# pansanity666/TransHuman

Measured on AMD Instinct MI355X. Metric: rays/sec (512x512, 64 samples/ray), higher is better.
Workload: dtype f32 (fp16 hi/lo x3 MFMA emulation)

## Files before the change

transhuman_amd/csrc/k_mlp_fused8_kernel.h:

```cpp
#pragma once
#include "k_mlp_fused_kernel.h"

typedef float f8_f4 __attribute__((ext_vector_type(4)));
typedef short f8_s4 __attribute__((ext_vector_type(4)));
typedef short f8_s8 __attribute__((ext_vector_type(8)));

#define F8_THREADS 512
#define F8_PART_FLOATS (3 * 8 * 32)
#define F8_PSTR 12
#define F8_MISC_FLOATS (F8_PSTR * 32 + F8_PART_FLOATS + 32 + 8)
#define F8_LDS_BYTES (ABUF_BYTES + MBUF_BYTES + F8_MISC_FLOATS * 4)
static_assert(F8_LDS_BYTES <= 163840, "the 8-wave tile must fit the CU's LDS");

#define F8_MFMA(A, B, C) __builtin_amdgcn_mfma_f32_16x16x32_f16((A), (B), (C), 0, 0, 0)

template <int CT>
__device__ __forceinline__ void f8_load_w(const uint4* __restrict__ wl, int t, uint4 (&w)[CT][2]) {
    const uint4* p = wl + (long long)t * (CT * 2 * 64);
#pragma unroll
    for (int c = 0; c < CT; ++c) {
        w[c][0] = p[(c * 2 + 0) * 64];
        w[c][1] = p[(c * 2 + 1) * 64];
    }
}
#define F8_WSLICE(L, wave, ct) ((L).w + (long long)(wave) * (L).KB * ((ct) * 2 * 64))

template <int NR, int ROWSTEP, bool PERM>
__device__ __forceinline__ void f8_load_x(const char* __restrict__ ahi, const char* __restrict__ alo, int aoff, int t,
                                          h8 (&xh)[NR], h8 (&xl)[NR]) {
    const int ko = (PERM ? 32 : 64) * t;
#pragma unroll
    for (int r = 0; r < NR; ++r) {
        xh[r] = *reinterpret_cast<const h8*>(ahi + r * ROWSTEP + aoff + ko);
        xl[r] = *reinterpret_cast<const h8*>(alo + r * ROWSTEP + aoff + ko);
    }
}
template <bool PERM>
__device__ __forceinline__ int f8_aoff(int lane, int str) {
    const int l = lane & 15, g = lane >> 4;
    return PERM ? l * str + 16 * (g >> 1) + 256 * (g & 1) : l * str + 16 * g;
}

template <int CT, int RT, int NR, int R0, bool FIRST>
__device__ __forceinline__ void f8_mfma_half(const uint4 (&w)[CT][2], const h8 (&xh)[NR], const h8 (&xl)[NR], f8_f4 (&acc)[CT][RT]) {
    const f8_f4 zero = {0.f, 0.f, 0.f, 0.f};
#pragma unroll
    for (int c = 0; c < CT; ++c)
#pragma unroll
        for (int r = 0; r < NR; ++r)
            acc[c][R0 + r] = F8_MFMA(*reinterpret_cast<const h8*>(&w[c][1]), xh[r], FIRST ? zero : acc[c][R0 + r]);
#pragma unroll
    for (int c = 0; c < CT; ++c)
#pragma unroll
        for (int r = 0; r < NR; ++r) acc[c][R0 + r] = F8_MFMA(*reinterpret_cast<const h8*>(&w[c][0]), xl[r], acc[c][R0 + r]);
#pragma unroll
    for (int c = 0; c < CT; ++c)
#pragma unroll
        for (int r = 0; r < NR; ++r) acc[c][R0 + r] = F8_MFMA(*reinterpret_cast<const h8*>(&w[c][0]), xh[r], acc[c][R0 + r]);
}

template <int NMEM, int NMF>
__device__ __forceinline__ void f8_interleave() {
    constexpr int NP = NMEM < NMF ? NMEM : NMF;
#pragma unroll
    for (int q = 0; q < NP; ++q) {
        __builtin_amdgcn_sched_group_barrier(0x008, 1, 0);
        __builtin_amdgcn_sched_group_barrier(0x120, 1, 0);
    }
    if constexpr (NMF > NP) __builtin_amdgcn_sched_group_barrier(0x008, NMF - NP, 0);
    if constexpr (NMEM > NP) __builtin_amdgcn_sched_group_barrier(0x120, NMEM - NP, 0);
    FM_SB();
}

template <int RT, int CT, int ROWSTEP, bool PERM, bool PRE = false>
__device__ __forceinline__ void f8_gemm(const char* __restrict__ ahi, const char* __restrict__ alo, int str,
                                        const uint4* __restrict__ wp, int T, int lane, f8_f4 (&acc)[CT][RT], uint4 (&w)[2][CT][2]) {
    static_assert(RT % 2 == 0, "row tiles come in halves");
    constexpr int NR = RT / 2;
    const uint4* wl = wp + lane;
    const int aoff = f8_aoff<PERM>(lane, str);
    h8 xah[NR], xal[NR], xbh[NR], xbl[NR];
    if (!PRE) f8_load_w<CT>(wl, 0, w[0]);
    f8_load_x<NR, ROWSTEP, PERM>(ahi, alo, aoff, 0, xah, xal);
    FM_SB();
    auto step = [&](auto first, auto par, int t) __attribute__((always_inline)) {
        constexpr bool F = decltype(first)::value;
        constexpr int PB = decltype(par)::value;
        const int tn = t + 1 < T ? t + 1 : T - 1;
        f8_load_x<NR, ROWSTEP, PERM>(ahi + NR * ROWSTEP, alo + NR * ROWSTEP, aoff, t, xbh, xbl);
        f8_load_w<CT>(wl, tn, w[PB ^ 1]);
        f8_mfma_half<CT, RT, NR, 0, F>(w[PB], xah, xal, acc);
        f8_interleave<2 * NR + 2 * CT, 3 * CT * NR>();
        f8_load_x<NR, ROWSTEP, PERM>(ahi, alo, aoff, tn, xah, xal);
        f8_mfma_half<CT, RT, NR, NR, F>(w[PB], xbh, xbl, acc);
        f8_interleave<2 * NR, 3 * CT * NR>();
    };
    step(std::true_type{}, std::integral_constant<int, 0>{}, 0);
    if (T > 1) {
        step(std::false_type{}, std::integral_constant<int, 1>{}, 1);
#pragma unroll 1
        for (int t = 2; t < T; t += 2) {
            step(std::false_type{}, std::integral_constant<int, 0>{}, t);
            step(std::false_type{}, std::integral_constant<int, 1>{}, t + 1);
        }
    }
}

template <int RT, int CT, int ROWSTEP, bool PERM, bool PRE = false>
__device__ __forceinline__ void f8_gemm3(const char* __restrict__ ahi, const char* __restrict__ alo, int str,
                                         const uint4* __restrict__ wp, int T, int lane, f8_f4 (&acc)[CT][RT], uint4 (&w)[2][CT][2]) {
    static_assert(RT % 3 == 0, "row tiles come in thirds");
    constexpr int NR = RT / 3;
    const uint4* wl = wp + lane;
    const int aoff = f8_aoff<PERM>(lane, str);
    h8 xh[2][NR], xl[2][NR];
    if (!PRE) f8_load_w<CT>(wl, 0, w[0]);
    f8_load_x<NR, ROWSTEP, PERM>(ahi, alo, aoff, 0, xh[0], xl[0]);
    FM_SB();
    auto sub = [&](auto first, auto sidx, int t) __attribute__((always_inline)) {
        constexpr int S = decltype(sidx)::value, G = S % 3, PB = S / 3, CUR = S & 1;
        constexpr bool F = decltype(first)::value && S < 3;
        constexpr int GN = (G + 1) % 3;
        const int tt = t + PB;
        const int tx = G == 2 ? (tt + 1 < T ? tt + 1 : T - 1) : tt;
        f8_load_x<NR, ROWSTEP, PERM>(ahi + GN * NR * ROWSTEP, alo + GN * NR * ROWSTEP, aoff, tx, xh[CUR ^ 1], xl[CUR ^ 1]);
        if constexpr (G == 0) f8_load_w<CT>(wl, tt + 1 < T ? tt + 1 : T - 1, w[PB ^ 1]);
        f8_mfma_half<CT, RT, NR, G * NR, F>(w[PB], xh[CUR], xl[CUR], acc);
        f8_interleave<2 * NR + (G == 0 ? 2 * CT : 0), 3 * CT * NR>();
    };
    auto pair = [&](auto first, int t) __attribute__((always_inline)) {
        sub(first, std::integral_constant<int, 0>{}, t); sub(first, std::integral_constant<int, 1>{}, t);
        sub(first, std::integral_constant<int, 2>{}, t); sub(first, std::integral_constant<int, 3>{}, t);
        sub(first, std::integral_constant<int, 4>{}, t); sub(first, std::integral_constant<int, 5>{}, t);
    };
    pair(std::true_type{}, 0);
#pragma unroll 1
    for (int t = 2; t < T; t += 2) pair(std::false_type{}, t);
}
template <int RT, int CT, int ROWSTEP, bool PERM, bool PRE = false>
__device__ __forceinline__ void f8_gemm_rt(const char* __restrict__ ahi, const char* __restrict__ alo, int str,
                                           const uint4* __restrict__ wp, int T, int lane, f8_f4 (&acc)[CT][RT], uint4 (&w)[2][CT][2]) {
    if constexpr (RT % 3 == 0) f8_gemm3<RT, CT, ROWSTEP, PERM, PRE>(ahi, alo, str, wp, T, lane, acc, w);
    else f8_gemm<RT, CT, ROWSTEP, PERM, PRE>(ahi, alo, str, wp, T, lane, acc, w);
}

template <int STR, bool NONNEG = true>
__device__ __forceinline__ void f8_store_h(const f8_f4& t, int row, int col0, char* __restrict__ hi, char* __restrict__ lo, int lane,
                                           unsigned& rm) {
    const int c = col0 + 4 * (lane >> 4);
    uint2 a, b;
    split_pair(t[0], t[1], a.x, b.x);
    split_pair(t[2], t[3], a.y, b.y);
    range_acc<NONNEG>(rm, a.x);
    range_acc<NONNEG>(rm, a.y);
    *reinterpret_cast<uint2*>(hi + row * STR + 2 * c) = a;
    *reinterpret_cast<uint2*>(lo + row * STR + 2 * c) = b;
}
__device__ __forceinline__ f8_f4 f8_finish(const f8_f4& a, const float4& b, float inv_scale, bool relu) {
    const f32x2 sc = {inv_scale, inv_scale};
    f32x2 y01 = __builtin_elementwise_fma((f32x2){a[0], a[1]}, sc, (f32x2){b.x, b.y});
    f32x2 y23 = __builtin_elementwise_fma((f32x2){a[2], a[3]}, sc, (f32x2){b.z, b.w});
    if (relu) {
        y01 = __builtin_elementwise_max(y01, (f32x2){0.f, 0.f});
        y23 = __builtin_elementwise_max(y23, (f32x2){0.f, 0.f});
    }
    return (f8_f4){y01[0], y01[1], y23[0], y23[1]};
}
__device__ __forceinline__ float f8_xor(float v, int lane, int mask) {
    return __builtin_bit_cast(float, __builtin_amdgcn_ds_bpermute((lane ^ mask) << 2, __builtin_bit_cast(int, v)));
}
__device__ __forceinline__ float4 f8_bias(const float* __restrict__ bias, int col0, int lane) {
    return *reinterpret_cast<const float4*>(bias + col0 + 4 * (lane >> 4));
}

template <int RT, int NV, int H, int R0, bool FIRST>
__device__ __forceinline__ void f8_mfma_dual(const uint4 (&r3)[2][2], const uint4 (&ra)[1][2], const h8 (&mh)[1], const h8 (&ml)[1],
                                             const h8 (&xh)[NV], const h8 (&xl)[NV], f8_f4 (&a3)[2][2], f8_f4 (&va)[1][RT]) {
    const f8_f4 zero = {0.f, 0.f, 0.f, 0.f};
#pragma unroll
    for (int t = 0; t < 3; ++t) {
        const int wp = t == 0 ? 1 : 0;
        const bool lo = t == 1;
        const bool first = FIRST && t == 0;
        a3[0][H] = F8_MFMA(*reinterpret_cast<const h8*>(&r3[0][wp]), lo ? ml[0] : mh[0], first ? zero : a3[0][H]);
#pragma unroll
        for (int r = 0; r < NV; ++r) {
            va[0][R0 + r] = F8_MFMA(*reinterpret_cast<const h8*>(&ra[0][wp]), lo ? xl[r] : xh[r], first ? zero : va[0][R0 + r]);
            if (r == 0) a3[1][H] = F8_MFMA(*reinterpret_cast<const h8*>(&r3[1][wp]), lo ? ml[0] : mh[0], first ? zero : a3[1][H]);
        }
    }
}

template <int V>
__global__ __launch_bounds__(F8_THREADS, 2) void mlp_fused8_kernel(FusedParams P_arg) {
#define PK P_arg
    struct F8Dbg { long long* dbg; };
    const F8Dbg P{PK.dbg};
    extern __shared__ __attribute__((aligned(16))) char lds[];
    char* abuf = lds;
    char* mbuf = lds + ABUF_BYTES;
    float* misc = reinterpret_cast<float*>(lds + ABUF_BYTES + MBUF_BYTES);
    float* probs = misc;
    float* part = misc + F8_PSTR * 32;
    float* sig = part + F8_PART_FLOATS;
    int* flag = reinterpret_cast<int*>(sig + 32);

    const int tid = threadIdx.x, lane = tid & 63, wave = tid >> 6;
    const int l15 = lane & 15, g4 = lane >> 4;
    const int tile = (int)((blockIdx.x & 7) * (gridDim.x >> 3) + (blockIdx.x >> 3));
    const int pbase = tile * FM_PTS;
    if (pbase >= PK.P) return;
    const int npts = min(FM_PTS, PK.P - pbase);
    const int fm_dbg_tile = tile;
    const int zoff = 0;
    constexpr int ROWS = 32 * V, RT = 2 * V;
    constexpr int RS256 = 16 * STR256;
    int dbg_i = 1;
    long long dbg_t = 0;
    long long* dbg_keep = reinterpret_cast<long long*>(flag + 2);
    constexpr float inv_v = 1.0f / (float)V;
    unsigned rmax = 0u;
    unsigned seen_s = 0u, seen_p = 0u, seen_n = 0u, seen_i = 0u, seen_4 = 0u;
    char* a256_lo = abuf + ROWS * STR256;

    struct TexPre { unsigned h0, h1; fm_u4 rq; };
    auto tex_fetch = [&]() __attribute__((always_inline)) {
        int tl = tile;
        asm volatile("" : "+s"(tl));
        TexPre t;
        const unsigned* hb = PK.tex_hdr + (long long)tl * 512;
        t.h0 = hb[lane];
        t.h1 = hb[64 + lane];
        t.rq = (fm_u4){0u, 0u, 0u, 0u};
        if (tid < 64 * V) t.rq = *reinterpret_cast<const fm_u4*>(PK.tex_rec + (long long)tl * V * 32 * 8 + tid * 4);
        return t;
    };
    auto fill_tex = [&](const TexPre& pre, auto rgb, auto&& under) __attribute__((always_inline)) {
        constexpr bool RGB = decltype(rgb)::value;
        constexpr int TSTR = 1040, TMAX = 103, NK = (TMAX + 7) / 8, NR = 4 * V;
        static_assert(TMAX * TSTR <= ABUF_BYTES, "a pass of texel rows must fit the operand buffer");
        int wv = __builtin_amdgcn_readfirstlane(wave), tl = tile;
        asm volatile("" : "+s"(wv), "+s"(tl));
        const unsigned* hb = PK.tex_hdr + (long long)tl * 512;
        unsigned h0 = pre.h0, h1 = pre.h1;
        const int npass = __builtin_amdgcn_readfirstlane((int)(h0 >> 16));
        char* recl = reinterpret_cast<char*>(misc);
        static_assert(32 * V * 32 <= (F8_PSTR * 32 + F8_PART_FLOATS) * 4, "row records must fit probs + part");
        unsigned fv[NR][4] = {};
        f32x2 bias_lo = {0.f, 0.f}, bias_hi = {0.f, 0.f};
        if constexpr (!RGB) {
            const float4 b4 = *reinterpret_cast<const float4*>(PK.ar0.bias + 4 * lane);
            bias_lo = (f32x2){b4.x, b4.y};
            bias_hi = (f32x2){b4.z, b4.w};
        }
        for (int p = 0; p < npass; ++p) {
            if (p > 0) {
                FM_SYNCL();
                h0 = hb[p * 128 + lane];
                h1 = hb[p * 128 + 64 + lane];
            }
            const int U = __builtin_amdgcn_readfirstlane((int)(h0 & 0xffffu));
            {
                constexpr int NA = 7, NB = 10;
                const char* mbase = reinterpret_cast<const char*>(RGB ? PK.tex_map2 : PK.tex_map);
                const unsigned loff = (unsigned)lane * 16u;
                const int last = U - 1;
                fm_u4 ta[NA], tb[NB - NA], tc[NK - NB];
#pragma unroll
                for (int k = 0; k < NA; ++k) {
                    const int i = min(wv + 8 * k, last);
                    const unsigned id = (unsigned)__builtin_amdgcn_readlane((int)h0, 8 + i);
                    ta[k] = *reinterpret_cast<const fm_u4*>(mbase + TX_ADDR(id));
                }
                const bool more = U > 8 * NA, most = U > 8 * NB;
                if (more) {
#pragma unroll
                    for (int k = NA; k < NB; ++k) {
                        const int i = min(wv + 8 * k, last);
                        const unsigned id = (unsigned)__builtin_amdgcn_readlane((int)h1, i - 56);
                        tb[k - NA] = *reinterpret_cast<const fm_u4*>(mbase + TX_ADDR(id));
                    }
                }
                if (most) {
#pragma unroll
                    for (int k = NB; k < NK; ++k) {
                        const int i = min(wv + 8 * k, last);
                        const unsigned id = (unsigned)__builtin_amdgcn_readlane((int)h1, i - 56);
                        tc[k - NB] = *reinterpret_cast<const fm_u4*>(mbase + TX_ADDR(id));
                    }
                }
                if (p == 0) {
                    under();
                    if (tid < 64 * V) *reinterpret_cast<fm_u4*>(recl + tid * 16) = pre.rq;
                }
                int wv2 = wv;
                asm volatile("" : "+s"(wv2));
#pragma unroll
                for (int k = 0; k < NA; ++k) *reinterpret_cast<fm_u4*>(abuf + min(wv2 + 8 * k, last) * TSTR + lane * 16) = ta[k];
                if (more) {
#pragma unroll
                    for (int k = NA; k < NB; ++k) *reinterpret_cast<fm_u4*>(abuf + min(wv2 + 8 * k, last) * TSTR + lane * 16) = tb[k - NA];
                }
                if (most) {
#pragma unroll
                    for (int k = NB; k < NK; ++k) *reinterpret_cast<fm_u4*>(abuf + min(wv2 + 8 * k, last) * TSTR + lane * 16) = tc[k - NB];
                }
            }
            FM_SYNCL();
            const int sh2 = npass == 1 ? 2 : npass == 2 ? 1 : 0;
            const int cofs = lane * 16;
            struct RowIn { float4 a, b, c, d; fm_u4 q0; };
            auto issue = [&](int k, const fm_u4& o, RowIn& r) __attribute__((always_inline)) {
                r.q0 = *reinterpret_cast<const fm_u4*>(recl + (wv + 8 * k) * 32);
                r.a = *reinterpret_cast<const float4*>(abuf + (o[0] + cofs));
                r.b = *reinterpret_cast<const float4*>(abuf + (o[1] + cofs));
                r.c = *reinterpret_cast<const float4*>(abuf + (o[2] + cofs));
                r.d = *reinterpret_cast<const float4*>(abuf + (o[3] + cofs));
            };
            auto offs = [&](int k) __attribute__((always_inline)) {
                return *reinterpret_cast<const fm_u4*>(recl + (wv + 8 * k) * 32 + 16);
            };
            auto blend = [&](int k, const RowIn& r, auto sel) __attribute__((always_inline)) {
                const unsigned u0 = r.q0[0], u1 = r.q0[1], u2 = r.q0[2], u3 = r.q0[3];
                const float w00 = __builtin_bit_cast(float, u0), w01 = __builtin_bit_cast(float, u1),
                            w10 = __builtin_bit_cast(float, u2), w11 = __builtin_bit_cast(float, u3);
                const f32x2 W00 = {w00, w00}, W01 = {w01, w01}, W10 = {w10, w10}, W11 = {w11, w11};
                f32x2 lo = (f32x2){r.a.x, r.a.y} * W00, hi = (f32x2){r.a.z, r.a.w} * W00;
                lo = __builtin_elementwise_fma((f32x2){r.b.x, r.b.y}, W01, lo);
                hi = __builtin_elementwise_fma((f32x2){r.b.z, r.b.w}, W01, hi);
                lo = __builtin_elementwise_fma((f32x2){r.c.x, r.c.y}, W10, lo);
                hi = __builtin_elementwise_fma((f32x2){r.c.z, r.c.w}, W10, hi);
                lo = __builtin_elementwise_fma((f32x2){r.d.x, r.d.y}, W11, lo);
                hi = __builtin_elementwise_fma((f32x2){r.d.z, r.d.w}, W11, hi);
                unsigned n0, n1, n2, n3;
                if constexpr (RGB) {
                    const float l0 = lo[0], l1 = lo[1], h0f = hi[0], h1f = hi[1];
                    n0 = __builtin_bit_cast(unsigned, l0); n1 = __builtin_bit_cast(unsigned, l1);
                    n2 = __builtin_bit_cast(unsigned, h0f); n3 = __builtin_bit_cast(unsigned, h1f);
                } else {
                    lo = __builtin_elementwise_max(lo + bias_lo, (f32x2){0.f, 0.f});
                    hi = __builtin_elementwise_max(hi + bias_hi, (f32x2){0.f, 0.f});
                    split_pair(lo[0], lo[1], n0, n2);
                    split_pair(hi[0], hi[1], n1, n3);
                }
                if constexpr (decltype(sel)::value) {
                    const bool mine = ((k & 3) >> sh2) == p;
                    fv[k][0] = mine ? n0 : fv[k][0]; fv[k][1] = mine ? n1 : fv[k][1];
                    fv[k][2] = mine ? n2 : fv[k][2]; fv[k][3] = mine ? n3 : fv[k][3];
                } else {
                    fv[k][0] = n0; fv[k][1] = n1; fv[k][2] = n2; fv[k][3] = n3;
                }
            };
            auto rows_loop = [&](auto sel) __attribute__((always_inline)) {
                RowIn in[2];
                fm_u4 of[2];
                of[0] = offs(0);
                of[1] = offs(1);
                issue(0, of[0], in[0]);
#pragma unroll
                for (int k = 0; k < NR; ++k) {
                    if (k + 1 < NR) issue(k + 1, of[(k + 1) & 1], in[(k + 1) & 1]);
                    if (k + 2 < NR) of[k & 1] = offs(k + 2);
                    FM_SB();
                    blend(k, in[k & 1], sel);
                    FM_SB();
                }
            };
            if (npass == 1) rows_loop(std::false_type{});
            else rows_loop(std::true_type{});
        }
        FM_SYNCL();
        if constexpr (RGB) {
#pragma unroll
            for (int k = 0; k < NR; ++k)
                *reinterpret_cast<fm_u4*>(abuf + (wv + 8 * k) * TSTR + lane * 16) = (fm_u4){fv[k][0], fv[k][1], fv[k][2], fv[k][3]};
        } else {
#pragma unroll
            for (int k = 0; k < NR; ++k) {
                range_acc<true>(rmax, fv[k][0]);
                range_acc<true>(rmax, fv[k][1]);
                *reinterpret_cast<uint2*>(abuf + (wv + 8 * k) * STR256 + lane * 8) = make_uint2(fv[k][0], fv[k][1]);
                *reinterpret_cast<uint2*>(a256_lo + (wv + 8 * k) * STR256 + lane * 8) = make_uint2(fv[k][2], fv[k][3]);
            }
            range_commit(PK.range, TH_RANGE_P, seen_p, rmax);
        }
    };

    if (PK.dbg != nullptr && tid == 0 && (tile & 15) == 0) {
        atomicAdd(reinterpret_cast<unsigned long long*>(PK.dbg), 1ull);
        dbg_t = clock64();
        dbg_keep[0] = dbg_t;
        dbg_keep[1] = wall_clock64();
    }
    fm_u4 rv4 = {0u, 0u, 0u, 0u};
    unsigned rv1 = 0u;
    static_assert(TH_RANGE_S == 1 && TH_RANGE_P == 2 && TH_RANGE_N == 3 && TH_RANGE_INTER == 4 && TH_RANGE_F4 == 5, "range slots 1..5");
    if (PK.range != nullptr) {
        const unsigned* rtab = PK.range + zoff;
        rv4 = (fm_u4){rtab[1], rtab[2], rtab[3], rtab[4]};
        rv1 = rtab[5];
    }
    TexPre tex_pre = tex_fetch(), tex_pre2;

    int vsel[2] = {0, 0};
    float vdv[2] = {0.f, 0.f};
    f8_f4 acc2[2][RT];
    {
        constexpr int STOK_STR = 1040;
        static_assert(32 * V * STOK_STR <= ABUF_BYTES, "T' rows must fit the operand buffer");
        char* pe_hi = mbuf;
        char* pe_lo = mbuf + 32 * STR64;
        const int pt = tid & 255, prow = pt >> 3, pc = pt & 7, ppl = tid >> 8;
        const int psrc = min(prow, npts - 1);
        const uint4 pe_v = *reinterpret_cast<const uint4*>(PK.pe + (long long)(pbase + psrc) * 128 + 64 * ppl + 8 * pc);
        char* wsp_hi = mbuf + 16384;
        char* wsp_lo = wsp_hi + 32 * STRVD;
        const unsigned* hdr = reinterpret_cast<const unsigned*>(PK.stok) + (long long)((PK.P + 31) / 32 * 32) * 16 + (long long)tile * 128;
        const unsigned h0 = hdr[lane], h1 = hdr[64 + lane];
        const int ns = tid / 7, nk = tid - 7 * ns;
        int slot = -1;
        float nw = 0.f;
        if (tid < 224) {
            const unsigned* rec = reinterpret_cast<const unsigned*>(PK.stok) + (long long)(pbase + min(ns, npts - 1)) * 16;
            slot = (int)rec[nk];
            nw = __builtin_bit_cast(float, rec[8 + nk]);
        }
        const unsigned zq = 0u;
        const float inv_t = PK.t_inv[zoff];
        uint4 wq[2][2][2];
        const uint4* wl = F8_WSLICE(PK.w16.fc_0pe, wave, 2) + lane;
        f8_load_w<2>(wl, 0, wq[0]);
        f8_load_w<2>(wl, 1, wq[1]);
        const float4 b0[2] = {f8_bias(PK.fc_0pe.bias, wave * 32, lane), f8_bias(PK.fc_0pe.bias, wave * 32 + 16, lane)};
        if (tid < 2 * 32 * STRVD / 16) reinterpret_cast<uint4*>(wsp_hi)[tid] = make_uint4(zq, zq, zq, zq);
        *reinterpret_cast<uint4*>((ppl ? pe_lo : pe_hi) + prow * STR64 + 16 * pc) = pe_v;
        const int U = __builtin_amdgcn_readfirstlane((int)h0);
        FM_SB();
        auto slot_centre = [&](int u) {
            const int d = (2 + u) >> 1;
            const unsigned src = d < 64 ? (unsigned)__builtin_amdgcn_readlane((int)h0, d) : (unsigned)__builtin_amdgcn_readlane((int)h1, d - 64);
            return (int)((src >> (16 * ((2 + u) & 1))) & 0xffffu);
        };
#pragma unroll
        for (int c = 0; c < 2; ++c)
#pragma unroll
            for (int r = 0; r < RT; ++r) acc2[c][r] = (f8_f4){0.f, 0.f, 0.f, 0.f};
        f8_f4 a1[2][2] = {{{0.f, 0.f, 0.f, 0.f}, {0.f, 0.f, 0.f, 0.f}}, {{0.f, 0.f, 0.f, 0.f}, {0.f, 0.f, 0.f, 0.f}}};
        const int wv = __builtin_amdgcn_readfirstlane(wave);
        const int aoffw = f8_aoff<false>(lane, STRVD), aoffp = f8_aoff<false>(lane, STR64);
        for (int u0 = 0; u0 < U; u0 += 32) {
            const int nU = min(32, U - u0);
            if (u0 > 0) {
                FM_SYNCL();
                if (tid < 2 * 32 * STRVD / 16) reinterpret_cast<uint4*>(wsp_hi)[tid] = make_uint4(zq, zq, zq, zq);
            }
            for (int u = wv; u < nU; u += 8) {
                const int cu = slot_centre(u0 + u);
                const char* g = reinterpret_cast<const char*>(PK.tsplit) + (long long)cu * 1024 + lane * 16;
#pragma unroll
                for (int vw = 0; vw < V; ++vw)
                    __builtin_amdgcn_global_load_lds((fm_gptr)(g + (long long)vw * PK.t_nc * 1024),
                                                     (fm_lptr)(abuf + (vw * 32 + u) * STOK_STR), 16, 0, 0);
            }
            FM_SYNCL();
            if (slot >= u0 && slot < u0 + 32) {
                _Float16 hi, lo;
                split_h(nw, hi, lo);
                *reinterpret_cast<_Float16*>(wsp_hi + ns * STRVD + 2 * (slot - u0)) = hi;
                *reinterpret_cast<_Float16*>(wsp_lo + ns * STRVD + 2 * (slot - u0)) = lo;
            }
            if (u0 == 0) {
#pragma unroll
                for (int t = 0; t < 2; ++t) {
                    h8 xh[2], xl[2];
                    f8_load_x<2, 16 * STR64, false>(pe_hi, pe_lo, aoffp, t, xh, xl);
                    if (t == 0) f8_mfma_half<2, 2, 2, 0, true>(wq[0], xh, xl, a1);
                    else f8_mfma_half<2, 2, 2, 0, false>(wq[1], xh, xl, a1);
                }
            }
            FM_SYNC();
            {
                h8 xh[2], xl[2];
                f8_load_x<2, 16 * STRVD, false>(wsp_hi, wsp_lo, aoffw, 0, xh, xl);
                const int tq = l15 >> 2, tc = 8 * (l15 & 3);
                const int ro0 = min(8 * g4 + tq, nU - 1) * STOK_STR + tc, ro1 = min(8 * g4 + 4 + tq, nU - 1) * STOK_STR + tc;
                typedef __attribute__((address_space(3))) f8_s4* f8_lp;
#pragma unroll
                for (int r = 0; r < V; ++r)
#pragma unroll
                    for (int c = 0; c < 2; ++c) {
                        const char* rb = abuf + r * 32 * STOK_STR + 2 * (wave * 32 + c * 16);
                        const f8_s4 h0 = __builtin_amdgcn_ds_read_tr16_b64_v4i16((f8_lp)(rb + ro0));
                        const f8_s4 h1 = __builtin_amdgcn_ds_read_tr16_b64_v4i16((f8_lp)(rb + ro1));
                        const f8_s4 l0 = __builtin_amdgcn_ds_read_tr16_b64_v4i16((f8_lp)(rb + ro0 + 512));
                        const f8_s4 l1 = __builtin_amdgcn_ds_read_tr16_b64_v4i16((f8_lp)(rb + ro1 + 512));
                        const f8_s8 ahs = __builtin_shufflevector(h0, h1, 0, 1, 2, 3, 4, 5, 6, 7);
                        const f8_s8 als = __builtin_shufflevector(l0, l1, 0, 1, 2, 3, 4, 5, 6, 7);
                        const h8 ah = __builtin_bit_cast(h8, ahs), al = __builtin_bit_cast(h8, als);
#pragma unroll
                        for (int h = 0; h < 2; ++h) {
                            acc2[c][2 * r + h] = F8_MFMA(al, xh[h], acc2[c][2 * r + h]);
                            acc2[c][2 * r + h] = F8_MFMA(ah, xl[h], acc2[c][2 * r + h]);
                            acc2[c][2 * r + h] = F8_MFMA(ah, xh[h], acc2[c][2 * r + h]);
                        }
                    }
            }
        }
        FM_SYNCL();
        {
            asm volatile("" : "+v"(rv4), "+v"(rv1));
            seen_s = (unsigned)__builtin_amdgcn_readfirstlane((int)rv4[0]);
            seen_p = (unsigned)__builtin_amdgcn_readfirstlane((int)rv4[1]);
            seen_n = (unsigned)__builtin_amdgcn_readfirstlane((int)rv4[2]);
            seen_i = (unsigned)__builtin_amdgcn_readfirstlane((int)rv4[3]);
            seen_4 = (unsigned)__builtin_amdgcn_readfirstlane((int)rv1);
        }
#pragma unroll
        for (int c = 0; c < 2; ++c) {
            f8_f4 pe2[2];
#pragma unroll
            for (int h = 0; h < 2; ++h) pe2[h] = f8_finish(a1[c][h], b0[c], PK.fc_0pe.inv_scale, false);
#pragma unroll
            for (int r = 0; r < RT; ++r) {
                const f32x2 it2 = {inv_t, inv_t};
                f32x2 u01 = __builtin_elementwise_fma((f32x2){acc2[c][r][0], acc2[c][r][1]}, it2, (f32x2){pe2[r & 1][0], pe2[r & 1][1]});
                f32x2 u23 = __builtin_elementwise_fma((f32x2){acc2[c][r][2], acc2[c][r][3]}, it2, (f32x2){pe2[r & 1][2], pe2[r & 1][3]});
                u01 = __builtin_elementwise_max(u01, (f32x2){0.f, 0.f});
                u23 = __builtin_elementwise_max(u23, (f32x2){0.f, 0.f});
                const f8_f4 u = {u01[0], u01[1], u23[0], u23[1]};
                f8_store_h<STR256>(u, r * 16 + l15, wave * 32 + c * 16, abuf, a256_lo, lane, rmax);
            }
        }
        range_commit(PK.range, TH_RANGE_S, seen_s, rmax);
    }
    uint4 wk3[2][3][2];
    FM_SB();
    f8_load_w<3>(F8_WSLICE(PK.w16.kv1, wave, 3) + lane, 0, wk3[0]);
    FM_SYNCL();
    f8_f4 vs[2][RT];
    float* ksb = reinterpret_cast<float*>(mbuf);
    {
        f8_f4 acc3[3][RT];
        f8_gemm_rt<RT, 3, RS256, true, true>(abuf, a256_lo, STR256, F8_WSLICE(PK.w16.kv1, wave, 3), 8, lane, acc3, wk3);
        const float4 bk = f8_bias(PK.kv1.bias, wave * 16, lane), bv0 = f8_bias(PK.kv1.bias, 128 + wave * 32, lane),
                     bv1 = f8_bias(PK.kv1.bias, 128 + wave * 32 + 16, lane);
#pragma unroll
        for (int r = 0; r < RT; ++r) {
            const f8_f4 k = f8_finish(acc3[0][r], bk, PK.kv1.inv_scale, false);
            *reinterpret_cast<float4*>(ksb + (r * 16 + l15) * KSTR + wave * 16 + 4 * g4) = make_float4(k[0], k[1], k[2], k[3]);
            vs[0][r] = f8_finish(acc3[1][r], bv0, PK.kv1.inv_scale, false);
            vs[1][r] = f8_finish(acc3[2][r], bv1, PK.kv1.inv_scale, false);
        }
    }
    FM_SYNCL();

    FM_SB();
    fill_tex(tex_pre, std::false_type{}, [] {});
    FM_SB();
    f8_load_w<3>(F8_WSLICE(PK.w16.kv0, wave, 3) + lane, 0, wk3[0]);
    FM_SYNCL();
    f8_f4 vp[2][RT];
    {
        f8_f4 acc3[3][RT];
        f8_gemm_rt<RT, 3, RS256, true, true>(abuf, a256_lo, STR256, F8_WSLICE(PK.w16.kv0, wave, 3), 8, lane, acc3, wk3);
        const float4 bk = f8_bias(PK.kv0.bias, wave * 16, lane), bv0 = f8_bias(PK.kv0.bias, 128 + wave * 32, lane),
                     bv1 = f8_bias(PK.kv0.bias, 128 + wave * 32 + 16, lane);
        FM_SYNCL();
        float* kpb = reinterpret_cast<float*>(abuf);
#pragma unroll
        for (int r = 0; r < RT; ++r) {
            const f8_f4 k = f8_finish(acc3[0][r], bk, PK.kv0.inv_scale, false);
            *reinterpret_cast<float4*>(kpb + (r * 16 + l15) * KSTR + wave * 16 + 4 * g4) = make_float4(k[0], k[1], k[2], k[3]);
            vp[0][r] = f8_finish(acc3[1][r], bv0, PK.kv0.inv_scale, false);
            vp[1][r] = f8_finish(acc3[2][r], bv1, PK.kv0.inv_scale, false);
        }
    }
    FM_SYNCL();

    {
        const float* kpb = reinterpret_cast<const float*>(abuf);
        float4 bn[2];
        {
            const int p = tid >> 4, c16 = tid & 15;
            f32x2 acc2[V * V];
#pragma unroll
            for (int ji = 0; ji < V * V; ++ji) acc2[ji] = (f32x2){0.f, 0.f};
#pragma unroll
            for (int q = 0; q < 2; ++q) {
                float4 kx[V], sx[V];
#pragma unroll
                for (int v = 0; v < V; ++v) {
                    kx[v] = *reinterpret_cast<const float4*>(kpb + (v * 32 + p) * KSTR + 4 * (c16 + 16 * q));
                    sx[v] = *reinterpret_cast<const float4*>(ksb + (v * 32 + p) * KSTR + 4 * (c16 + 16 * q));
                }
#pragma unroll
                for (int j = 0; j < V; ++j)
#pragma unroll
                    for (int i = 0; i < V; ++i) {
                        acc2[j * V + i] = __builtin_elementwise_fma((f32x2){kx[j].x, kx[j].y}, (f32x2){sx[i].x, sx[i].y}, acc2[j * V + i]);
                        acc2[j * V + i] = __builtin_elementwise_fma((f32x2){kx[j].z, kx[j].w}, (f32x2){sx[i].z, sx[i].w}, acc2[j * V + i]);
                    }
            }
            float acc[V * V];
#pragma unroll
            for (int ji = 0; ji < V * V; ++ji) {
                float s = acc2[ji][0] + acc2[ji][1];
                s += __builtin_bit_cast(float, __builtin_amdgcn_update_dpp(0, __builtin_bit_cast(int, s), 0xB1, 0xF, 0xF, true));
                s += __builtin_bit_cast(float, __builtin_amdgcn_update_dpp(0, __builtin_bit_cast(int, s), 0x4E, 0xF, 0xF, true));
                s += __builtin_bit_cast(float, __builtin_amdgcn_update_dpp(0, __builtin_bit_cast(int, s), 0x141, 0xF, 0xF, true));
                s += __builtin_bit_cast(float, __builtin_amdgcn_update_dpp(0, __builtin_bit_cast(int, s), 0x140, 0xF, 0xF, true));
                acc[ji] = s;
            }
            float a[V], m = -3.0e38f;
#pragma unroll
            for (int j = 0; j < V; ++j) {
                float x = acc[j * V];
#pragma unroll
                for (int i = 1; i < V; ++i) x = c16 == i ? acc[j * V + i] : x;
                a[j] = x / 11.313708498984761f;
                m = fmaxf(m, a[j]);
            }
            float e[V], se = 0.f;
#pragma unroll
            for (int j = 0; j < V; ++j) { e[j] = expf(a[j] - m); se = se + e[j]; }
            if (c16 < V) {
#pragma unroll
                for (int j = 0; j < V; ++j) probs[p * F8_PSTR + j * V + c16] = e[j] / se;
            }
        }
        bn[0] = f8_bias(PK.fc_1.bias, wave * 32, lane);
        bn[1] = f8_bias(PK.fc_1.bias, wave * 32 + 16, lane);
        FM_SYNCL();
#pragma unroll
        for (int h = 0; h < 2; ++h) {
            const float* pr = probs + (h * 16 + l15) * F8_PSTR;
            const float4 q0 = *reinterpret_cast<const float4*>(pr), q1 = *reinterpret_cast<const float4*>(pr + 4);
            const float q2 = pr[8];
            const float A[9] = {q0.x, q0.y, q0.z, q0.w, q1.x, q1.y, q1.z, q1.w, q2};
#pragma unroll
            for (int c = 0; c < 2; ++c) {
                const f32x2 b01 = {bn[c].x, bn[c].y}, b23 = {bn[c].z, bn[c].w};
                f32x2 t0[V], t1[V];
#pragma unroll
                for (int i = 0; i < V; ++i) {
                    t0[i] = (f32x2){vs[c][2 * i + h][0], vs[c][2 * i + h][1]} + b01;
                    t1[i] = (f32x2){vs[c][2 * i + h][2], vs[c][2 * i + h][3]} + b23;
                }
#pragma unroll
                for (int j = 0; j < V; ++j) {
                    const f32x2 v0 = {vp[c][2 * j + h][0], vp[c][2 * j + h][1]}, v1 = {vp[c][2 * j + h][2], vp[c][2 * j + h][3]};
#pragma unroll
                    for (int i = 0; i < V; ++i) {
                        const f32x2 a2 = {A[j * V + i], A[j * V + i]};
                        t0[i] = __builtin_elementwise_fma(v0, a2, t0[i]);
                        t1[i] = __builtin_elementwise_fma(v1, a2, t1[i]);
                    }
                }
#pragma unroll
                for (int i = 0; i < V; ++i) {
                    t0[i] = __builtin_elementwise_max(t0[i], (f32x2){0.f, 0.f});
                    t1[i] = __builtin_elementwise_max(t1[i], (f32x2){0.f, 0.f});
                    const f8_f4 n = {t0[i][0], t0[i][1], t1[i][0], t1[i][1]};
                    f8_store_h<STR256>(n, (2 * i + h) * 16 + l15, wave * 32 + c * 16, abuf, a256_lo, lane, rmax);
                }
            }
        }
        range_commit(PK.range, TH_RANGE_N, seen_n, rmax);
    }

    uint4 wk2[2][2][2];
    FM_SB();
    f8_load_w<2>(F8_WSLICE(PK.w16.fc_2, wave, 2) + lane, 0, wk2[0]);
#pragma unroll
    for (int q = 0; q < 2; ++q) {
        const int i = tid + F8_THREADS * q, row = i >> 5, c = i & 31;
        int x = pbase + row;
        if (PK.vd_sel != nullptr && PK.rgb_all != 2 && c < 27 && row < npts) x = PK.vd_sel[pbase + row];
        vsel[q] = x;
    }
    FM_SYNCL();
    f8_gemm_rt<RT, 2, RS256, true, true>(abuf, a256_lo, STR256, F8_WSLICE(PK.w16.fc_2, wave, 2), 8, lane, acc2, wk2);
    const float4 bi[2] = {f8_bias(PK.fc_2.bias, wave * 32, lane), f8_bias(PK.fc_2.bias, wave * 32 + 16, lane)};
#pragma unroll
    for (int q = 0; q < 2; ++q) {
        const int i = tid + F8_THREADS * q, row = i >> 5, c = i & 31;
        float x = 0.f;
        if (PK.rgb_all != 2 && c < 27 && row < npts) {
            const long long vr = PK.vd_sel ? (long long)(vsel[q] / PK.vd_div) : (long long)(pbase + row);
            x = PK.vd[vr * 27 + c];
        }
        vdv[q] = x;
    }
    FM_SYNCL();
#pragma unroll
    for (int c = 0; c < 2; ++c) {
#pragma unroll
        for (int r = 0; r < RT; ++r) acc2[c][r] = f8_finish(acc2[c][r], bi[c], PK.fc_2.inv_scale, true);
#pragma unroll
        for (int h = 0; h < 2; ++h) {
            f8_f4 m = acc2[c][h];
#pragma unroll
            for (int r = 1; r < V; ++r) m = m + acc2[c][2 * r + h];
            m = m * (f8_f4){inv_v, inv_v, inv_v, inv_v};
            f8_store_h<STR256>(m, h * 16 + l15, wave * 32 + c * 16, mbuf, mbuf + 32 * STR256, lane, rmax);
        }
#pragma unroll
        for (int r = 0; r < RT; ++r) f8_store_h<STR256>(acc2[c][r], r * 16 + l15, wave * 32 + c * 16, abuf, a256_lo, lane, rmax);
    }
    range_commit(PK.range, TH_RANGE_INTER, seen_i, rmax);
    FM_SYNCL();

    char* vd_hi = mbuf + MBUF_VD_OFF;
    char* vd_lo = vd_hi + 32 * STRVD;
    tex_pre2 = tex_fetch();
    f8_f4 va[1][RT];
    {
        f8_f4 a3[2][2];
        const float4 aw[2] = {f8_bias(PK.alpha_w, wave * 32, lane), f8_bias(PK.alpha_w, wave * 32 + 16, lane)};
        const float4 b3[2] = {f8_bias(PK.fc_3.bias, wave * 32, lane), f8_bias(PK.fc_3.bias, wave * 32 + 16, lane)};
        if (PK.rgb_all != 2) {
            constexpr int T = 8;
            const uint4* w3l = F8_WSLICE(PK.w16.fc_3, wave, 2) + lane;
            const uint4* wal = F8_WSLICE(PK.w16.vfA, wave, 1) + lane;
            const int aoff = f8_aoff<true>(lane, STR256);
            const char* mhi = mbuf;
            const char* mlo = mbuf + 32 * STR256;
            uint4 r3[2][2][2], ra[2][1][2];
            h8 mah[1], mal[1], xah[V], xal[V], mbh[1], mbl[1], xbh[V], xbl[V];
            f8_load_w<2>(w3l, 0, r3[0]);
            f8_load_w<1>(wal, 0, ra[0]);
            f8_load_x<1, RS256, true>(mhi, mlo, aoff, 0, mah, mal);
            f8_load_x<V, RS256, true>(abuf, a256_lo, aoff, 0, xah, xal);
            FM_SB();
            auto step = [&](auto first, auto par, int t) __attribute__((always_inline)) {
                constexpr bool F = decltype(first)::value;
                constexpr int PB = decltype(par)::value;
                const int tn = t + 1 < T ? t + 1 : T - 1;
                f8_load_x<1, RS256, true>(mhi + RS256, mlo + RS256, aoff, t, mbh, mbl);
                f8_load_x<V, RS256, true>(abuf + V * RS256, a256_lo + V * RS256, aoff, t, xbh, xbl);
                f8_load_w<2>(w3l, tn, r3[PB ^ 1]);
                f8_load_w<1>(wal, tn, ra[PB ^ 1]);
                f8_mfma_dual<RT, V, 0, 0, F>(r3[PB], ra[PB], mah, mal, xah, xal, a3, va);
                f8_interleave<2 + 2 * V + 6, 3 * (2 + V)>();
                f8_load_x<1, RS256, true>(mhi, mlo, aoff, tn, mah, mal);
                f8_load_x<V, RS256, true>(abuf, a256_lo, aoff, tn, xah, xal);
                f8_mfma_dual<RT, V, 1, V, F>(r3[PB], ra[PB], mbh, mbl, xbh, xbl, a3, va);
                f8_interleave<2 + 2 * V, 3 * (2 + V)>();
            };
            step(std::true_type{}, std::integral_constant<int, 0>{}, 0);
            step(std::false_type{}, std::integral_constant<int, 1>{}, 1);
#pragma unroll 1
            for (int t = 2; t < T; t += 2) {
                step(std::false_type{}, std::integral_constant<int, 0>{}, t);
                step(std::false_type{}, std::integral_constant<int, 1>{}, t + 1);
            }
        } else {
#pragma unroll
            for (int r = 0; r < RT; ++r) va[0][r] = (f8_f4){0.f, 0.f, 0.f, 0.f};
            uint4 w3[2][2][2];
            f8_gemm<2, 2, RS256, true, false>(mbuf, mbuf + 32 * STR256, STR256, F8_WSLICE(PK.w16.fc_3, wave, 2), 8, lane, a3, w3);
        }
        float s2[2];
#pragma unroll
        for (int h = 0; h < 2; ++h) {
            float s = 0.f;
#pragma unroll
            for (int c = 0; c < 2; ++c) {
                const f8_f4 y = f8_finish(a3[c][h], b3[c], PK.fc_3.inv_scale, true);
                s = fmaf(y[0], aw[c].x, s);
                s = fmaf(y[1], aw[c].y, s);
                s = fmaf(y[2], aw[c].z, s);
                s = fmaf(y[3], aw[c].w, s);
            }
            s += f8_xor(s, lane, 16);
            s += f8_xor(s, lane, 32);
            s2[h] = s;
        }
        if (g4 == 0) part[wave * 32 + l15] = s2[0];
        if (g4 == 1) part[wave * 32 + 16 + l15] = s2[1];
        if (tid == 0) *flag = 0;
        FM_SYNCL();
        if (tid < 32) {
            float sg = PK.alpha_b[zoff];
#pragma unroll
            for (int w = 0; w < 8; ++w) sg += part[w * 32 + tid];
            sig[tid] = sg;
            if (tid < npts && PK.rgb_all != 2 && (PK.rgb_all == 1 || sg > 0.f)) *flag = 1;
        }
#pragma unroll
        for (int q = 0; q < 2; ++q) {
            const int i = tid + F8_THREADS * q, row = i >> 5, c = i & 31;
            _Float16 a, b;
            split_h(vdv[q], a, b);
            *reinterpret_cast<_Float16*>(vd_hi + row * STRVD + 2 * c) = a;
            *reinterpret_cast<_Float16*>(vd_lo + row * STRVD + 2 * c) = b;
        }
        FM_SYNCL();
    }
    const bool need_rgb = *flag != 0;
    float rgb_out[3] = {0.f, 0.f, 0.f};
    if (need_rgb) {
        uint4 wvd[1][2];
        f8_load_w<1>(F8_WSLICE(PK.w16.vfD, wave, 1) + lane, 0, wvd);
        FM_SB();
        fill_tex(tex_pre2, std::true_type{}, [&]() __attribute__((always_inline)) {
            h8 xh[2], xl[2];
            f8_load_x<2, 16 * STRVD, false>(vd_hi, vd_lo, f8_aoff<false>(lane, STRVD), 0, xh, xl);
#pragma unroll
            for (int r = 0; r < RT; ++r) {
                va[0][r] = F8_MFMA(*reinterpret_cast<const h8*>(&wvd[0][1]), xh[r & 1], va[0][r]);
                va[0][r] = F8_MFMA(*reinterpret_cast<const h8*>(&wvd[0][0]), xl[r & 1], va[0][r]);
                va[0][r] = F8_MFMA(*reinterpret_cast<const h8*>(&wvd[0][0]), xh[r & 1], va[0][r]);
            }
        });
        FM_SYNCL();
        uint4 w4[4][1][2];
        {
            const uint4* wl4 = F8_WSLICE(PK.w16.fc_4, wave, 1) + lane;
#pragma unroll
            for (int t = 0; t < 4; ++t) f8_load_w<1>(wl4, t, w4[t]);
        }
        float4 rw[3];
#pragma unroll
        for (int o = 0; o < 3; ++o) rw[o] = f8_bias(PK.rgb_w + o * 128, wave * 16, lane);
        const float4 b4 = f8_bias(PK.fc_4.bias, wave * 16, lane);
        const float4 bt = f8_bias(PK.rst.bias, wave * 16, lane), br = f8_bias(PK.rst.bias, 128 + wave * 16, lane);
        char* f4_hi = mbuf + MBUF_FC4_OFF;
        char* f4_lo = f4_hi + 32 * STR128;
        {
            const char* mb = abuf + l15 * 1040 + 4 * (wave * 16 + 4 * g4);
            f8_f4 u[RT];
#pragma unroll
            for (int r = 0; r < RT; ++r) {
                const float4 m1 = *reinterpret_cast<const float4*>(mb + r * 16 * 1040);
                const float4 m2 = *reinterpret_cast<const float4*>(mb + r * 16 * 1040 + 512);
                const f8_f4 t = f8_finish(va[0][r], bt, PK.rst.inv_scale, false);
                const f32x2 z2 = {0.f, 0.f};
                const f32x2 u01 = __builtin_elementwise_max((f32x2){t[0], t[1]} + (f32x2){m1.x, m1.y}, z2) + ((f32x2){m2.x, m2.y} + (f32x2){br.x, br.y});
                const f32x2 u23 = __builtin_elementwise_max((f32x2){t[2], t[3]} + (f32x2){m1.z, m1.w}, z2) + ((f32x2){m2.z, m2.w} + (f32x2){br.z, br.w});
                u[r] = (f8_f4){u01[0], u01[1], u23[0], u23[1]};
            }
#pragma unroll
            for (int h = 0; h < 2; ++h) {
                f8_f4 m = u[h];
#pragma unroll
                for (int r = 1; r < V; ++r) m = m + u[2 * r + h];
                m = m * (f8_f4){inv_v, inv_v, inv_v, inv_v};
                f8_store_h<STR128, false>(m, h * 16 + l15, wave * 16, f4_hi, f4_lo, lane, rmax);
            }
            range_commit(PK.range, TH_RANGE_F4, seen_4, rmax);
        }
        FM_SYNCL();
        f8_f4 a4[1][2];
        {
            const int aoff4 = f8_aoff<false>(lane, STR128);
#pragma unroll
            for (int t = 0; t < 4; ++t) {
                h8 xh4[2], xl4[2];
                f8_load_x<2, 16 * STR128, false>(f4_hi, f4_lo, aoff4, t, xh4, xl4);
                if (t == 0) f8_mfma_half<1, 2, 2, 0, true>(w4[t], xh4, xl4, a4);
                else f8_mfma_half<1, 2, 2, 0, false>(w4[t], xh4, xl4, a4);
            }
        }
        float s3[3][2];
#pragma unroll
        for (int h = 0; h < 2; ++h) {
            const f8_f4 y = f8_finish(a4[0][h], b4, PK.fc_4.inv_scale, true);
#pragma unroll
            for (int o = 0; o < 3; ++o) {
                float s = 0.f;
                s = fmaf(y[0], rw[o].x, s);
                s = fmaf(y[1], rw[o].y, s);
                s = fmaf(y[2], rw[o].z, s);
                s = fmaf(y[3], rw[o].w, s);
                s += f8_xor(s, lane, 16);
                s += f8_xor(s, lane, 32);
                s3[o][h] = s;
            }
        }
#pragma unroll
        for (int o = 0; o < 3; ++o) {
            if (g4 == 0) part[(o * 8 + wave) * 32 + l15] = s3[o][0];
            if (g4 == 1) part[(o * 8 + wave) * 32 + 16 + l15] = s3[o][1];
        }
        FM_SYNCL();
        if (tid < 32) {
#pragma unroll
            for (int o = 0; o < 3; ++o) {
                float s = PK.rgb_b[zoff + o];
#pragma unroll
                for (int w = 0; w < 8; ++w) s += part[(o * 8 + w) * 32 + tid];
                rgb_out[o] = s;
            }
        }
    }
    if (tid < npts)
        *reinterpret_cast<float4*>(PK.raw_c + (long long)(pbase + tid) * 4) = make_float4(rgb_out[0], rgb_out[1], rgb_out[2], sig[tid]);
    if (FM_DBG_SAMPLED) {
        atomicAdd(reinterpret_cast<unsigned long long*>(P.dbg + 62), (unsigned long long)(clock64() - dbg_keep[0]));
        atomicAdd(reinterpret_cast<unsigned long long*>(P.dbg + 63), (unsigned long long)(wall_clock64() - dbg_keep[1]));
    }
#undef PK
}
```

Baseline: 18.89 million.

## Move attention scores to MFMA, use permlane reductions, prefetch fc_3 weights

The K projections are now stored as fp16 hi/lo splits, and the VxV attention score dot products are computed with MFMA on a subset of waves rather than with scalar FMAs plus DPP reductions. Cross-lane sums in the alpha and rgb heads use permlane16/32 swaps instead of ds_bpermute, folding two halves per call. The first four fc_3 weight tiles are prefetched into registers before the sync, and the fc_4 loop is split into two independent accumulator chains. These changes add register pressure and introduce fp16-split rounding into the attention scores, and only some waves do the score work.

```diff
diff --git a/transhuman_amd/csrc/k_mlp_fused8_kernel.h b/transhuman_amd/csrc/k_mlp_fused8_kernel.h
--- a/transhuman_amd/csrc/k_mlp_fused8_kernel.h
+++ b/transhuman_amd/csrc/k_mlp_fused8_kernel.h
@@ -37,6 +37,7 @@
 }
 template <bool PERM>
 __device__ __forceinline__ int f8_aoff(int lane, int str) {
+    asm volatile("" : "+v"(lane));
     const int l = lane & 15, g = lane >> 4;
     return PERM ? l * str + 16 * (g >> 1) + 256 * (g & 1) : l * str + 16 * g;
 }
@@ -166,8 +167,11 @@
     }
     return (f8_f4){y01[0], y01[1], y23[0], y23[1]};
 }
-__device__ __forceinline__ float f8_xor(float v, int lane, int mask) {
-    return __builtin_bit_cast(float, __builtin_amdgcn_ds_bpermute((lane ^ mask) << 2, __builtin_bit_cast(int, v)));
+__device__ __forceinline__ float f8_fold2(float a, float b) {
+    const auto p = __builtin_amdgcn_permlane16_swap(__builtin_bit_cast(unsigned, a), __builtin_bit_cast(unsigned, b), false, false);
+    const float u = __builtin_bit_cast(float, p[0]) + __builtin_bit_cast(float, p[1]);
+    const auto q = __builtin_amdgcn_permlane32_swap(__builtin_bit_cast(unsigned, u), __builtin_bit_cast(unsigned, u), false, false);
+    return __builtin_bit_cast(float, q[0]) + __builtin_bit_cast(float, q[1]);
 }
 __device__ __forceinline__ float4 f8_bias(const float* __restrict__ bias, int col0, int lane) {
     return *reinterpret_cast<const float4*>(bias + col0 + 4 * (lane >> 4));
@@ -538,7 +542,7 @@
     f8_load_w<3>(F8_WSLICE(PK.w16.kv1, wave, 3) + lane, 0, wk3[0]);
     FM_SYNCL();
     f8_f4 vs[2][RT];
-    float* ksb = reinterpret_cast<float*>(mbuf);
+    char* ksh = mbuf;
     {
         f8_f4 acc3[3][RT];
         f8_gemm_rt<RT, 3, RS256, true, true>(abuf, a256_lo, STR256, F8_WSLICE(PK.w16.kv1, wave, 3), 8, lane, acc3, wk3);
@@ -547,10 +551,15 @@
 #pragma unroll
         for (int r = 0; r < RT; ++r) {
             const f8_f4 k = f8_finish(acc3[0][r], bk, PK.kv1.inv_scale, false);
-            *reinterpret_cast<float4*>(ksb + (r * 16 + l15) * KSTR + wave * 16 + 4 * g4) = make_float4(k[0], k[1], k[2], k[3]);
+            f8_store_h<STR256, false>(k, r * 16 + l15, wave * 16, ksh, ksh + 256, lane, rmax);
+        }
+        FM_SB();
+#pragma unroll
+        for (int r = 0; r < RT; ++r) {
             vs[0][r] = f8_finish(acc3[1][r], bv0, PK.kv1.inv_scale, false);
             vs[1][r] = f8_finish(acc3[2][r], bv1, PK.kv1.inv_scale, false);
         }
+        range_commit(PK.range, TH_RANGE_N, seen_n, rmax);
     }
     FM_SYNCL();
 
@@ -566,66 +575,63 @@
         const float4 bk = f8_bias(PK.kv0.bias, wave * 16, lane), bv0 = f8_bias(PK.kv0.bias, 128 + wave * 32, lane),
                      bv1 = f8_bias(PK.kv0.bias, 128 + wave * 32 + 16, lane);
         FM_SYNCL();
-        float* kpb = reinterpret_cast<float*>(abuf);
 #pragma unroll
         for (int r = 0; r < RT; ++r) {
             const f8_f4 k = f8_finish(acc3[0][r], bk, PK.kv0.inv_scale, false);
-            *reinterpret_cast<float4*>(kpb + (r * 16 + l15) * KSTR + wave * 16 + 4 * g4) = make_float4(k[0], k[1], k[2], k[3]);
+            f8_store_h<STR256, false>(k, r * 16 + l15, wave * 16, abuf, abuf + 256, lane, rmax);
+        }
+        FM_SB();
+#pragma unroll
+        for (int r = 0; r < RT; ++r) {
             vp[0][r] = f8_finish(acc3[1][r], bv0, PK.kv0.inv_scale, false);
             vp[1][r] = f8_finish(acc3[2][r], bv1, PK.kv0.inv_scale, false);
         }
+        range_commit(PK.range, TH_RANGE_N, seen_n, rmax);
     }
     FM_SYNCL();
 
     {
-        const float* kpb = reinterpret_cast<const float*>(abuf);
         float4 bn[2];
-        {
-            const int p = tid >> 4, c16 = tid & 15;
-            f32x2 acc2[V * V];
-#pragma unroll
-            for (int ji = 0; ji < V * V; ++ji) acc2[ji] = (f32x2){0.f, 0.f};
-#pragma unroll
-            for (int q = 0; q < 2; ++q) {
-                float4 kx[V], sx[V];
-#pragma unroll
-                for (int v = 0; v < V; ++v) {
-                    kx[v] = *reinterpret_cast<const float4*>(kpb + (v * 32 + p) * KSTR + 4 * (c16 + 16 * q));
-                    sx[v] = *reinterpret_cast<const float4*>(ksb + (v * 32 + p) * KSTR + 4 * (c16 + 16 * q));
-                }
-#pragma unroll
-                for (int j = 0; j < V; ++j)
-#pragma unroll
-                    for (int i = 0; i < V; ++i) {
-                        acc2[j * V + i] = __builtin_elementwise_fma((f32x2){kx[j].x, kx[j].y}, (f32x2){sx[i].x, sx[i].y}, acc2[j * V + i]);
-                        acc2[j * V + i] = __builtin_elementwise_fma((f32x2){kx[j].z, kx[j].w}, (f32x2){sx[i].z, sx[i].w}, acc2[j * V + i]);
-                    }
-            }
-            float acc[V * V];
-#pragma unroll
-            for (int ji = 0; ji < V * V; ++ji) {
-                float s = acc2[ji][0] + acc2[ji][1];
-                s += __builtin_bit_cast(float, __builtin_amdgcn_update_dpp(0, __builtin_bit_cast(int, s), 0xB1, 0xF, 0xF, true));
-                s += __builtin_bit_cast(float, __builtin_amdgcn_update_dpp(0, __builtin_bit_cast(int, s), 0x4E, 0xF, 0xF, true));
-                s += __builtin_bit_cast(float, __builtin_amdgcn_update_dpp(0, __builtin_bit_cast(int, s), 0x141, 0xF, 0xF, true));
-                s += __builtin_bit_cast(float, __builtin_amdgcn_update_dpp(0, __builtin_bit_cast(int, s), 0x140, 0xF, 0xF, true));
-                acc[ji] = s;
-            }
+        const int wv = __builtin_amdgcn_readfirstlane(wave);
+        if (wv < 2 * V) {
+            const int i = wv >> 1, h = wv & 1;
+            int ln = lane;
+            asm volatile("" : "+v"(ln));
+            const int l15 = ln & 15, g4 = ln >> 4;
+            const char* ksr = ksh + (i * 32 + h * 16) * STR256;
+            const char* kpr = abuf + h * 16 * STR256;
+            const int aoff = f8_aoff<false>(ln, STR256);
+            f8_f4 sc[V][1];
+#pragma unroll
+            for (int t = 0; t < 4; ++t) {
+                h8 xh[1], xl[1];
+                uint4 kw[V][2];
+                f8_load_x<1, 0, false>(ksr, ksr + 256, aoff, t, xh, xl);
+#pragma unroll
+                for (int j = 0; j < V; ++j) {
+                    kw[j][0] = *reinterpret_cast<const uint4*>(kpr + j * 32 * STR256 + aoff + 64 * t);
+                    kw[j][1] = *reinterpret_cast<const uint4*>(kpr + j * 32 * STR256 + 256 + aoff + 64 * t);
+                }
+                if (t == 0) f8_mfma_half<V, 1, 1, 0, true>(kw, xh, xl, sc);
+                else f8_mfma_half<V, 1, 1, 0, false>(kw, xh, xl, sc);
+            }
+            const int comp = l15 & 3;
             float a[V], m = -3.0e38f;
 #pragma unroll
             for (int j = 0; j < V; ++j) {
-                float x = acc[j * V];
-#pragma unroll
-                for (int i = 1; i < V; ++i) x = c16 == i ? acc[j * V + i] : x;
+                float x = sc[j][0][0];
+                x = comp == 1 ? sc[j][0][1] : x;
+                x = comp == 2 ? sc[j][0][2] : x;
+                x = comp == 3 ? sc[j][0][3] : x;
                 a[j] = x / 11.313708498984761f;
                 m = fmaxf(m, a[j]);
             }
             float e[V], se = 0.f;
 #pragma unroll
             for (int j = 0; j < V; ++j) { e[j] = expf(a[j] - m); se = se + e[j]; }
-            if (c16 < V) {
-#pragma unroll
-                for (int j = 0; j < V; ++j) probs[p * F8_PSTR + j * V + c16] = e[j] / se;
+            if (g4 == (l15 >> 2)) {
+#pragma unroll
+                for (int j = 0; j < V; ++j) probs[(h * 16 + l15) * F8_PSTR + j * V + i] = e[j] / se;
             }
         }
         bn[0] = f8_bias(PK.fc_1.bias, wave * 32, lane);
@@ -691,6 +697,13 @@
         }
         vdv[q] = x;
     }
+    uint4 w3pre[4][2][2];
+    if (PK.rgb_all != 2) {
+        const uint4* w3l = F8_WSLICE(PK.w16.fc_3, wave, 2) + lane;
+#pragma unroll
+        for (int t = 0; t < 4; ++t) f8_load_w<2>(w3l, t, w3pre[t]);
+    }
+    FM_SB();
     FM_SYNCL();
 #pragma unroll
     for (int c = 0; c < 2; ++c) {
@@ -727,32 +740,35 @@
             const char* mlo = mbuf + 32 * STR256;
             uint4 r3[2][2][2], ra[2][1][2];
             h8 mah[1], mal[1], xah[V], xal[V], mbh[1], mbl[1], xbh[V], xbl[V];
-            f8_load_w<2>(w3l, 0, r3[0]);
             f8_load_w<1>(wal, 0, ra[0]);
             f8_load_x<1, RS256, true>(mhi, mlo, aoff, 0, mah, mal);
             f8_load_x<V, RS256, true>(abuf, a256_lo, aoff, 0, xah, xal);
             FM_SB();
-            auto step = [&](auto first, auto par, int t) __attribute__((always_inline)) {
+            auto step = [&](auto first, auto par, auto pre, int t) __attribute__((always_inline)) {
                 constexpr bool F = decltype(first)::value;
-                constexpr int PB = decltype(par)::value;
+                constexpr int PB = decltype(par)::value, PRE = decltype(pre)::value;
+                constexpr bool LD3 = PRE < 0 || PRE == 3;
                 const int tn = t + 1 < T ? t + 1 : T - 1;
                 f8_load_x<1, RS256, true>(mhi + RS256, mlo + RS256, aoff, t, mbh, mbl);
                 f8_load_x<V, RS256, true>(abuf + V * RS256, a256_lo + V * RS256, aoff, t, xbh, xbl);
-                f8_load_w<2>(w3l, tn, r3[PB ^ 1]);
+                if constexpr (LD3) f8_load_w<2>(w3l, tn, r3[PB ^ 1]);
                 f8_load_w<1>(wal, tn, ra[PB ^ 1]);
-                f8_mfma_dual<RT, V, 0, 0, F>(r3[PB], ra[PB], mah, mal, xah, xal, a3, va);
-                f8_interleave<2 + 2 * V + 6, 3 * (2 + V)>();
+                const uint4 (&w3)[2][2] = PRE >= 0 ? w3pre[PRE >= 0 ? PRE : 0] : r3[PB];
+                f8_mfma_dual<RT, V, 0, 0, F>(w3, ra[PB], mah, mal, xah, xal, a3, va);
+                f8_interleave<2 + 2 * V + (LD3 ? 6 : 2), 3 * (2 + V)>();
                 f8_load_x<1, RS256, true>(mhi, mlo, aoff, tn, mah, mal);
                 f8_load_x<V, RS256, true>(abuf, a256_lo, aoff, tn, xah, xal);
-                f8_mfma_dual<RT, V, 1, V, F>(r3[PB], ra[PB], mbh, mbl, xbh, xbl, a3, va);
+                f8_mfma_dual<RT, V, 1, V, F>(w3, ra[PB], mbh, mbl, xbh, xbl, a3, va);
                 f8_interleave<2 + 2 * V, 3 * (2 + V)>();
             };
-            step(std::true_type{}, std::integral_constant<int, 0>{}, 0);
-            step(std::false_type{}, std::integral_constant<int, 1>{}, 1);
+            step(std::true_type{}, std::integral_constant<int, 0>{}, std::integral_constant<int, 0>{}, 0);
+            step(std::false_type{}, std::integral_constant<int, 1>{}, std::integral_constant<int, 1>{}, 1);
+            step(std::false_type{}, std::integral_constant<int, 0>{}, std::integral_constant<int, 2>{}, 2);
+            step(std::false_type{}, std::integral_constant<int, 1>{}, std::integral_constant<int, 3>{}, 3);
 #pragma unroll 1
-            for (int t = 2; t < T; t += 2) {
-                step(std::false_type{}, std::integral_constant<int, 0>{}, t);
-                step(std::false_type{}, std::integral_constant<int, 1>{}, t + 1);
+            for (int t = 4; t < T; t += 2) {
+                step(std::false_type{}, std::integral_constant<int, 0>{}, std::integral_constant<int, -1>{}, t);
+                step(std::false_type{}, std::integral_constant<int, 1>{}, std::integral_constant<int, -1>{}, t + 1);
             }
         } else {
 #pragma unroll
@@ -772,12 +788,14 @@
                 s = fmaf(y[2], aw[c].z, s);
                 s = fmaf(y[3], aw[c].w, s);
             }
-            s += f8_xor(s, lane, 16);
-            s += f8_xor(s, lane, 32);
             s2[h] = s;
         }
-        if (g4 == 0) part[wave * 32 + l15] = s2[0];
-        if (g4 == 1) part[wave * 32 + 16 + l15] = s2[1];
+        const float s2t = f8_fold2(s2[0], s2[1]);
+        {
+            int ln = tid;
+            asm volatile("" : "+v"(ln));
+            if ((ln & 32) == 0) part[(ln >> 6) * 32 + (ln & 31)] = s2t;
+        }
         if (tid == 0) *flag = 0;
         FM_SYNCL();
         if (tid < 32) {
@@ -853,14 +871,23 @@
         FM_SYNCL();
         f8_f4 a4[1][2];
         {
+            f8_f4 a4b[1][2];
             const int aoff4 = f8_aoff<false>(lane, STR128);
 #pragma unroll
-            for (int t = 0; t < 4; ++t) {
-                h8 xh4[2], xl4[2];
+            for (int t = 0; t < 2; ++t) {
+                h8 xh4[2], xl4[2], xh5[2], xl5[2];
                 f8_load_x<2, 16 * STR128, false>(f4_hi, f4_lo, aoff4, t, xh4, xl4);
-                if (t == 0) f8_mfma_half<1, 2, 2, 0, true>(w4[t], xh4, xl4, a4);
-                else f8_mfma_half<1, 2, 2, 0, false>(w4[t], xh4, xl4, a4);
-            }
+                f8_load_x<2, 16 * STR128, false>(f4_hi, f4_lo, aoff4, t + 2, xh5, xl5);
+                if (t == 0) {
+                    f8_mfma_half<1, 2, 2, 0, true>(w4[0], xh4, xl4, a4);
+                    f8_mfma_half<1, 2, 2, 0, true>(w4[2], xh5, xl5, a4b);
+                } else {
+                    f8_mfma_half<1, 2, 2, 0, false>(w4[1], xh4, xl4, a4);
+                    f8_mfma_half<1, 2, 2, 0, false>(w4[3], xh5, xl5, a4b);
+                }
+            }
+            a4[0][0] = a4[0][0] + a4b[0][0];
+            a4[0][1] = a4[0][1] + a4b[0][1];
         }
         float s3[3][2];
 #pragma unroll
@@ -873,15 +900,15 @@
                 s = fmaf(y[1], rw[o].y, s);
                 s = fmaf(y[2], rw[o].z, s);
                 s = fmaf(y[3], rw[o].w, s);
-                s += f8_xor(s, lane, 16);
-                s += f8_xor(s, lane, 32);
                 s3[o][h] = s;
             }
         }
 #pragma unroll
         for (int o = 0; o < 3; ++o) {
-            if (g4 == 0) part[(o * 8 + wave) * 32 + l15] = s3[o][0];
-            if (g4 == 1) part[(o * 8 + wave) * 32 + 16 + l15] = s3[o][1];
+            const float t = f8_fold2(s3[o][0], s3[o][1]);
+            int ln = tid;
+            asm volatile("" : "+v"(ln));
+            if ((ln & 32) == 0) part[(o * 8 + (ln >> 6)) * 32 + (ln & 31)] = t;
         }
         FM_SYNCL();
         if (tid < 32) {
```

Measured after the change: 18.38 million. 0.973x the previous value.
